# gongaa/video-layout-generation

Hardware: AMD Instinct MI355X
Metric: training clips/sec at (B,T,N)=(32,16,64) d=256; 1/2/4/8-GPU scaling (higher is better)
Workload: dtype f32

## Files before the change

include/vlg_hip.h:

```cpp
#ifndef VLG_HIP_H
#define VLG_HIP_H

#include <stdint.h>

typedef uint16_t vlg_bf16;

#ifdef __cplusplus
extern "C" {
#endif

#define VLG_ERR_SHAPE   1001
#define VLG_ERR_ALIGN   1002

int         vlg_abi_version(void);
const char* vlg_build_arch(void);

#ifdef VLG_DIAG
void vlg_debug_set_clock_probe(unsigned long long* buf);
void vlg_debug_set_conv_probe(unsigned long long* buf);
void vlg_debug_set_gemm_bk(int bk);
void vlg_debug_set_gemm_run(int run);
#endif

int vlg_embed_fwd(const int64_t* slot_class, const float* slot_box,
// ... 16 lines not shown
int vlg_layernorm_bwd(const float* dy, const float* x, const float* mean, const float* rstd,
                      const float* gamma, const float* dres, float* dx_out,
                      float* slabs, int64_t slab_stride, int64_t slab_capacity,
                      int64_t rows, int d, void* stream);
int vlg_layernorm_bwd_bf16(const vlg_bf16* dy, const float* x, const float* mean, const float* rstd,
                           const float* gamma, const float* dres, float* dx_out,
                           float* slabs, int64_t slab_stride, int64_t slab_capacity,
                           int64_t rows, int d, void* stream);

#define VLG_EPI_NONE   0
#define VLG_EPI_BIAS   1
#define VLG_EPI_GELU   2
#define VLG_EPI_RESID  4
#define VLG_EPI_DGELU  8
#define VLG_EPI_BF16   16
#define VLG_EPI_SPLIT3 256
#define VLG_EPI_ACT_GELU 512
#define VLG_EPI_GELU_GRAD 1024
#define VLG_EPI_MUL    2048
#define VLG_EPI_A_BF16   32
#define VLG_EPI_B_BF16   64
#define VLG_EPI_OUT_BF16 128
int vlg_linear_fwd(const void* A, int lda, const void* W, int ldw, const float* bias,
                   void* C, int ldc, const void* aux_in, void* aux_out,
                   int64_t M, int N, int K, int epilogue, void* stream);
int vlg_linear_dgrad(const void* dY, int ldy, const void* W, int ldw,
                     void* dX, int ldx, const void* aux_in,
                     int64_t M, int N, int K, int epilogue, void* stream);
int vlg_linear_wgrad_slabs(int64_t M, int N, int K);
int vlg_linear_wgrad_slabs_for(int64_t M, int N, int K, int flags);
int vlg_linear_wgrad(const void* dY, int ldy, const void* X, int ldx,
                     float* slabs, int64_t slab_stride, int64_t slab_capacity,
                     int64_t M, int N, int K, int flags , void* stream);
int vlg_linear_dgrad_wgrad(const void* dY, int ldy, const void* W, int ldw, void* dX, int ldx, const void* aux_in,
                           const void* X, int ldxx, float* slabs, int64_t slab_stride, int64_t slab_capacity,
                           int64_t M, int N, int K, int epilogue,
                           const int64_t* rider_table , int rider_rows, void* stream);


int vlg_attention_fwd(const float* qkv, float* o, int64_t n_seq, int T, int d, void* stream);
int vlg_attention_bwd(const float* qkv, const float* dout, float* dqkv,
                      int64_t n_seq, int T, int d, void* stream);
int vlg_attention_fwd_bf16(const vlg_bf16* qkv, vlg_bf16* o, int64_t n_seq, int T, int d, void* stream);
int vlg_attention_bwd_bf16(const vlg_bf16* qkv, const vlg_bf16* dout, vlg_bf16* dqkv,
                           int64_t n_seq, int T, int d, void* stream);

int vlg_layout_loss_scratch(void);
int vlg_layout_loss(const float* out, int ld, const int64_t* tgt_class, const float* tgt_box,
                    const float* valid, float* dout, float* loss_out, float* scratch,
                    int B, int T, int N, int n_classes, float beta, float iou_eps,
                    float w_reg, float w_iou, float w_ce, void* stream);

int vlg_attention_clip_fwd(const float* qkv, const float* valid, float* out, float* lse,
                           int64_t B, int T, int N, int d, void* stream);
int vlg_attention_clip_bwd(const float* qkv, const float* valid, const float* out, const float* dout, const float* lse,
                           float* delta, float* dqkv, int64_t B, int T, int N, int d, void* stream);
int vlg_attention_clip_fwd_bf16(const vlg_bf16* qkv, const float* valid, vlg_bf16* out, float* lse,
                                int64_t B, int T, int N, int d, void* stream);
int vlg_attention_clip_bwd_bf16(const vlg_bf16* qkv, const float* valid, const vlg_bf16* out, const vlg_bf16* dout,
                                const float* lse, float* delta, vlg_bf16* dqkv,
                                int64_t B, int T, int N, int d, void* stream);

int vlg_reduce_slabs(const float* slabs, int64_t slab_stride, int n_slabs,
                     float* dst, int64_t len, void* stream);

int vlg_adam_step_graph(float* param, const float* grad, float* exp_avg, float* exp_avg_sq, vlg_bf16* shadow,
// ... 101 lines not shown
```

video-layout-generation_amd/csrc/gemm.hip:

```cpp
#include "common.h"
#include <type_traits>

#include "gemm_tile.h"
#include "reduce_body.h"

#define GEMM_A_GELU (1 << 20)
#define GEMM_B_GELU (1 << 21)
__device__ __forceinline__ float4 gelu4(float4 v) { return make_float4(gelu_f(v.x), gelu_f(v.y), gelu_f(v.z), gelu_f(v.w)); }

__device__ __forceinline__ __amdgpu_buffer_rsrc_t vlg_rsrc(const void* p, int bytes = 0x7fffffff) {
    return __builtin_amdgcn_make_buffer_rsrc(const_cast<void*>(p), 0, bytes, 0x00020000);
}

#ifndef VLG_EPI_PACE
#define VLG_EPI_PACE 0
#endif
#ifndef VLG_EPI_PACE_EVERY
#define VLG_EPI_PACE_EVERY 2
#endif
__device__ __forceinline__ void vlg_epi_pace(int issued) {
#if VLG_EPI_PACE > 0
    if (issued % VLG_EPI_PACE_EVERY == 0) __builtin_amdgcn_s_sleep(VLG_EPI_PACE);
#endif
}

#ifdef VLG_NO_SCHED_FENCE
#define VLG_SCHED_FENCE()
#else
#define VLG_SCHED_FENCE() __builtin_amdgcn_sched_barrier(0)
#endif

template <int BM, int BN, int BK, bool A_KC, bool B_KC>
constexpr int gemm_smem_floats() { return 2 * (Tile<BM, A_KC, BK>::FLOATS + Tile<BN, B_KC, BK>::FLOATS); }

template <int BM, int BN, int BK, bool A_KC, bool B_KC, int EPI, bool COLSUM>
__device__ __forceinline__ void gemm_f32_body(const GemmArgs& g, float* const smem, const int bid, const int nwg) {
    __builtin_amdgcn_s_setprio(3);
    using EO = float;
    const float* const gA = static_cast<const float*>(g.A);
    const float* const gB = static_cast<const float*>(g.B);
    const float* const gAuxIn = static_cast<const float*>(g.aux_in);
    float* const gAuxOut = static_cast<float*>(g.aux_out);
    constexpr int WM = (BM == BN && (BM == 128 || BM == 64)) ? 2 : (BM == 128 ? 4 : 1);
    constexpr int WN = 4 / WM;
    constexpr int TM = BM / (32 * WM), TN = BN / (32 * WN);
    constexpr int NCH = BK / 8;
    using TA = Tile<BM, A_KC, BK>;
    using TB = Tile<BN, B_KC, BK>;
    float* const As0 = smem;
    float* const Bs0 = smem + 2 * TA::FLOATS;

    const int q = nwg >> 3, rr = nwg & 7, xcd = bid & 7;
    const int swz = (xcd < rr ? xcd * (q + 1) : rr * (q + 1) + (xcd - rr) * q) + (bid >> 3);
    constexpr bool CHAIN = BM == 128 && BN == 128 && BK == 32 && !COLSUM && (EPI & ((1 << 20) | (1 << 21))) == 0;
    const int run = (CHAIN && g.run > 1) ? g.run : 1;
    const int tng = g.tiles_n / run;
    const int ntile = g.tiles_m * tng;
    const int split = swz / ntile;
    const int tile = swz - split * ntile;
    const int tm = tile / tng, tn = (tile - tm * tng) * run;
    const int64_t m0 = (int64_t)tm * BM;
    const int n0 = tn * BN;
    const int64_t kbeg = (int64_t)split * g.kc_per_split;
    int64_t kend = kbeg + g.kc_per_split;
    if (kend > g.Kc) kend = g.Kc;

// ... 255 lines not shown
                if (GUARD && col0 + j * 32 >= g.N) continue;
                float aux[16];
                if constexpr ((EPI & (VLG_EPI_RESID | VLG_EPI_DGELU | VLG_EPI_MUL)) != 0) {
#pragma unroll
                    for (int r = 0; r < 16; ++r) {
                        const int ro = i * 32 + (r & 3) + 8 * (r >> 2);
                        aux[r] = (!GUARD || row0 + ro < g.M) ? ld1(gAuxIn + base + ro * g.ldc + j * 32) : 0.f;
                    }
                }
#pragma unroll
                for (int r = 0; r < 16; ++r) {
                    const int ro = i * 32 + (r & 3) + 8 * (r >> 2);
                    if (GUARD && row0 + ro >= g.M) continue;
                    const int64_t o = base + ro * g.ldc + j * 32;
                    float v = acc[i][j][r];
                    if constexpr ((EPI & VLG_EPI_GELU) != 0) {
                        if constexpr ((EPI & VLG_EPI_GELU_GRAD) != 0) {
                            float c, pd;
                            gelu_parts(v, c, pd);
                            st1(gAuxOut + o, c + v * pd);
                            v *= c;
                        } else {
                            st1(gAuxOut + o, v);
                            v = gelu_f(v);
                        }
                    }
                    if constexpr ((EPI & VLG_EPI_RESID) != 0) v += aux[r];
                    if constexpr ((EPI & VLG_EPI_DGELU) != 0) v *= dgelu_f(aux[r]);
                    if constexpr ((EPI & VLG_EPI_MUL) != 0) v *= aux[r];
                    st1(Cs + o, v);
                }
            }
    };
    auto emit_fast = [&](int n0v) __attribute__((always_inline)) {
        const int64_t corner = m0 * g.ldc + n0v;
        const __amdgpu_buffer_rsrc_t dc = vlg_rsrc(Cs + corner);
        const __amdgpu_buffer_rsrc_t dxin = vlg_rsrc(gAuxIn ? gAuxIn + corner : gA);
        const __amdgpu_buffer_rsrc_t dxout = vlg_rsrc(gAuxOut ? gAuxOut + corner : Cs + corner);
        const int vc = ((wm * TM * 32 + 4 * h) * g.ldc + wn * TN * 32 + l31) * 4;
        const int rowb = g.ldc * 4;
        constexpr bool AUX = (EPI & (VLG_EPI_RESID | VLG_EPI_DGELU | VLG_EPI_MUL)) != 0;
        constexpr bool AUX_ALL = BK == 32;
        constexpr int NAUX = AUX_ALL ? TM * TN : 2;
        float auxb[NAUX][16];
        auto fetch = [&](float (&a)[16], int i, int j) __attribute__((always_inline)) {
#pragma unroll
            for (int r = 0; r < 16; ++r) {
                a[r] = __uint_as_float(__builtin_amdgcn_raw_buffer_load_b32(dxin, vc + j * 128, (i * 32 + (r & 3) + 8 * (r >> 2)) * rowb, 0));
                vlg_epi_pace(r + 1);
            }
        };
        if constexpr (AUX) {
            if constexpr (AUX_ALL) {
#pragma unroll
                for (int t = 0; t < TM * TN; ++t) fetch(auxb[t], t / TN, t % TN);
            } else {
                fetch(auxb[0], 0, 0);
            }
        }
#pragma unroll
        for (int i = 0; i < TM; ++i)
#pragma unroll
            for (int j = 0; j < TN; ++j) {
                const int tix = i * TN + j;
                float (&aux)[16] = auxb[AUX_ALL ? tix : (tix & 1)];
                if constexpr (AUX && !AUX_ALL) {
                    if (tix + 1 < TM * TN) fetch(auxb[(tix + 1) & 1], (tix + 1) / TN, (tix + 1) % TN);
// ... 12 lines not shown
                        vlg_epi_pace(2 * q + 2);
                    }
                } else if constexpr ((EPI & VLG_EPI_GELU) != 0) {
#pragma unroll
                    for (int q = 0; q < 8; ++q) {
                        __builtin_amdgcn_raw_buffer_store_b32(__float_as_uint(v[q].x), dxout, vc + j * 128, soff(2 * q), 0);
                        __builtin_amdgcn_raw_buffer_store_b32(__float_as_uint(v[q].y), dxout, vc + j * 128, soff(2 * q + 1), 0);
                        vlg_epi_pace(2 * q + 2);
                    }
                    gelu2n<8>(v);
                }
                if constexpr ((EPI & VLG_EPI_RESID) != 0) {
#pragma unroll
                    for (int q = 0; q < 8; ++q) v[q] += v2f{aux[2 * q], aux[2 * q + 1]};
                }
                if constexpr ((EPI & VLG_EPI_MUL) != 0) {
#pragma unroll
                    for (int q = 0; q < 8; ++q) v[q] *= v2f{aux[2 * q], aux[2 * q + 1]};
                }
                if constexpr ((EPI & VLG_EPI_DGELU) != 0) {
                    v2f u[8], d[8];
#pragma unroll
                    for (int q = 0; q < 8; ++q) u[q] = v2f{aux[2 * q], aux[2 * q + 1]};
                    dgelu2n<8>(u, d);
#pragma unroll
                    for (int q = 0; q < 8; ++q) v[q] *= d[q];
                }
#pragma unroll
                for (int q = 0; q < 8; ++q) {
                    __builtin_amdgcn_raw_buffer_store_b32(__float_as_uint(v[q].x), dc, vc + j * 128, soff(2 * q), 0);
                    __builtin_amdgcn_raw_buffer_store_b32(__float_as_uint(v[q].y), dc, vc + j * 128, soff(2 * q + 1), 0);
                    vlg_epi_pace(2 * q + 2);
                }
            }
    };
    if (fast_tile) {
        for (int rt = 0; rt < run; ++rt) {
            const int n0v = n0 + rt * BN;
            const bool has_next = rt + 1 < run;
            mainloop_fast(n0v, rt == 0, has_next);
            if (has_next) load_bias(n0v + BN);
            emit_fast(n0v);
            if (has_next) init_acc();
        }
    } else if (full) emit(std::false_type{});
    else emit(std::true_type{});
#ifdef VLG_TIMELINE
    if (g.clock_probe) {
        asm volatile("s_waitcnt vmcnt(0)" ::: "memory");
        const unsigned long long tl_exit = __builtin_amdgcn_s_memrealtime();
        if (tid == 0) {
            unsigned long long* o = g.clock_probe + 8 * (size_t)bid;
            o[0] = tl_entry; o[1] = tl_loop0; o[2] = tl_loop1; o[3] = tl_exit;
            o[4] = __builtin_amdgcn_s_getreg(4 | (31 << 11));
            o[5] = __builtin_amdgcn_s_getreg(20 | (31 << 11));
            o[6] = (unsigned long long)tile; o[7] = (unsigned long long)split;
        }
    }
#endif
    if constexpr (COLSUM) {
        static_assert(!A_KC, "column sums are taken from a contraction-major A tile");
        if (tn == 0) {
            constexpr int PR = TA::PER_ROW, NG = GEMM_THREADS / PR;
            float* red = smem;
            st4(red + (tid / PR) * BM + 4 * (tid % PR), make_float4(col_lo.x, col_lo.y, col_hi.x, col_hi.y));
            __syncthreads();
            if (tid < BM && m0 + tid < g.M) {
                float s = 0.f;
#pragma unroll 8
                for (int t = 0; t < NG; ++t) s += red[t * BM + tid];
                st1(Cs + g.colsum_off + m0 + tid, s);
            }
        }
    }
}

template <int BM, int BN, int BK, bool A_KC, bool B_KC, int EPI, bool COLSUM>
__global__ __launch_bounds__(GEMM_THREADS, (BM == 64 && BN == 64) ? 4 : (BK == 16 ? 3 : 2)) void gemm_f32_kernel(const GemmArgs g) {
    __shared__ __attribute__((aligned(16))) float smem[gemm_smem_floats<BM, BN, BK, A_KC, B_KC>()];
    gemm_f32_body<BM, BN, BK, A_KC, B_KC, EPI, COLSUM>(g, smem, (int)blockIdx.x, (int)gridDim.x);
}

template <int BT, int EPI_D>
__global__ __launch_bounds__(GEMM_THREADS, BT == 64 ? 4 : 2) void gemm_pair_kernel(const GemmArgs gd, const GemmArgs gw, const int nd, const int nd_pad,
                                                                                   const int nw, const int64_t* __restrict__ rider, const int rider_bpr) {
    constexpr int FD = gemm_smem_floats<BT, BT, 32, true, false>(), FW = gemm_smem_floats<BT, BT, 32, false, false>();
    __shared__ __attribute__((aligned(16))) float smem_all[FD > FW ? FD : FW];
    const int b = (int)blockIdx.x;
    if (b < nd_pad) {
        if (b < nd) gemm_f32_body<BT, BT, 32, true, false, EPI_D, false>(gd, smem_all, b, nd);
    } else if (b < nd_pad + nw) {
        gemm_f32_body<BT, BT, 32, false, false, VLG_EPI_NONE, true>(gw, smem_all, b - nd_pad, nw);
    } else {
        const int rb = b - nd_pad - nw;
        reduce_table_row(rider, rb / rider_bpr, rb % rider_bpr, rider_bpr, reinterpret_cast<float4(*)[16]>(smem_all));
    }
}

#ifdef VLG_DIAG
static unsigned long long* vlg_gemm_clock_probe = nullptr;
extern "C" void vlg_debug_set_clock_probe(unsigned long long* p) { vlg_gemm_clock_probe = p; }
#else
static constexpr unsigned long long* vlg_gemm_clock_probe = nullptr;
#endif

#ifdef VLG_DIAG
static int vlg_gemm_bk_forced = -1;
extern "C" void vlg_debug_set_gemm_bk(int bk) { vlg_gemm_bk_forced = (bk == 16 || bk == 32) ? bk : 0; }
#endif
static int gemm_bk_override() {
#ifdef VLG_DIAG
    if (vlg_gemm_bk_forced >= 0) return vlg_gemm_bk_forced;
#endif
    return VLG_TUNE("VLG_GEMM_BK", 0);
}

#ifdef VLG_DIAG
static int vlg_gemm_run_forced = -1;
extern "C" void vlg_debug_set_gemm_run(int run) { vlg_gemm_run_forced = run < 0 ? -1 : run; }
#else
static constexpr int vlg_gemm_run_forced = -1;
#endif
template <int BM, int BN, int BK, bool A_KC, bool B_KC>
static int gemm_run(const GemmArgs& g, int slots) {
    if (BM != 128 || BN != 128 || g.splits != 1) return 1;
    if (g.M % BM != 0 || g.N % BN != 0 || g.Kc % (2 * BK) != 0) return 1;
    const int64_t span_a = A_KC ? (int64_t)(BM - 1) * g.lda + g.Kc : g.Kc * g.lda + BM;
    const int64_t span_b = B_KC ? (int64_t)(2 * BN - 1) * g.ldb + g.Kc : g.Kc * g.ldb + 2 * BN;
    if (span_a >= (1ll << 28) || span_b >= (1ll << 28) || (int64_t)(BM - 1) * g.ldc + BN >= (1ll << 28)) return 1;
    if (vlg_gemm_run_forced == 0) return 1;
    int best = 1;
    for (int r = 2; r <= g.tiles_n; ++r)
        if (g.tiles_n % r == 0 && (int64_t)g.tiles_m * (g.tiles_n / r) >= slots) best = r;
    if (vlg_gemm_run_forced > 0 && g.tiles_n % vlg_gemm_run_forced == 0) best = vlg_gemm_run_forced;
    return best;
}

static bool gemm_small_tiles() { return VLG_TUNE("VLG_GEMM_SMALL", 1) != 0; }
static int gemm_small_below() { return VLG_TUNE("VLG_GEMM_SMALL_BELOW", 512); }
static int gemm_small_below_wgrad() { return VLG_TUNE("VLG_GEMM_SMALL_BELOW_WGRAD", 385); }
static bool gemm_wants_small(int64_t M, int N, int splits) {
    return gemm_small_tiles() && ((M + 127) / 128) * (int64_t)((N + 127) / 128) * splits < gemm_small_below();
}

template <int BM, int BN, bool A_KC, bool B_KC, int EPI, bool COLSUM>
static int launch_gemm(GemmArgs g, hipStream_t s) {
    if constexpr (BM == 128 && BN == 128 && !COLSUM && (EPI & (GEMM_A_GELU | GEMM_B_GELU)) == 0) {
        if (gemm_wants_small(g.M, g.N, g.splits)) return launch_gemm<64, 64, A_KC, B_KC, EPI, COLSUM>(g, s);
    }
    g.tiles_m = (int)((g.M + BM - 1) / BM);
    g.tiles_n = (g.N + BN - 1) / BN;
    g.run = 1;
    g.clock_probe = vlg_gemm_clock_probe;
    const dim3 block(GEMM_THREADS);
    constexpr bool CAN_RUN = BM == 128 && BN == 128 && !COLSUM && (EPI & (GEMM_A_GELU | GEMM_B_GELU)) == 0;
    if constexpr (BM == 128 && BN == 128) {
        const int forced = gemm_bk_override();
        const bool heavy_epilogue = (EPI & (VLG_EPI_GELU | VLG_EPI_DGELU)) != 0;
        int run32 = 1;
        if constexpr (CAN_RUN) run32 = gemm_run<BM, BN, 32, A_KC, B_KC>(g, 512);
        if (forced == 16 || (forced != 32 && heavy_epilogue && run32 == 1)) {
            const int64_t blocks = (int64_t)g.tiles_m * (g.tiles_n / g.run) * g.splits;
// ... 40 lines not shown
    if ((epilogue & VLG_EPI_BIAS) && !bias) return VLG_ERR_SHAPE;
    if ((epilogue & (VLG_EPI_RESID | VLG_EPI_DGELU)) && !aux_in) return VLG_ERR_SHAPE;
    if ((epilogue & VLG_EPI_GELU) && !aux_out) return VLG_ERR_SHAPE;
    if ((epilogue & VLG_EPI_MUL) != 0) return VLG_ERR_SHAPE;
    if ((epilogue & VLG_EPI_GELU_GRAD) && (split3 || epilogue != (VLG_EPI_BIAS | VLG_EPI_GELU | VLG_EPI_GELU_GRAD)))
        return VLG_ERR_SHAPE;
    const bool narrow = N <= 32;
    const bool act_gelu = (epilogue & VLG_EPI_ACT_GELU) != 0;
    epilogue &= ~VLG_EPI_ACT_GELU;
    if (act_gelu && (bf16 || split3)) return VLG_ERR_SHAPE;
    if (io != 0 && !bf16) return VLG_ERR_SHAPE;
    if (((io & 1) && (lda & 7)) || ((io & 2) && (ldw & 7))) return VLG_ERR_ALIGN;
    if (bf16) return vlg_gemm16_fwd(g, epilogue, io, s);
    if (split3) return vlg_gemm_split_fwd(g, epilogue, s);
    if (act_gelu) {
        if (epilogue != (VLG_EPI_BIAS | VLG_EPI_RESID) || narrow) return VLG_ERR_SHAPE;
        return launch_gemm<128, 128, true, true, VLG_EPI_BIAS | VLG_EPI_RESID | GEMM_A_GELU, false>(g, s);
    }
    switch (epilogue) {
        case VLG_EPI_BIAS:
            return narrow ? launch_gemm<128, 32, true, true, VLG_EPI_BIAS, false>(g, s)
                          : launch_gemm<128, 128, true, true, VLG_EPI_BIAS, false>(g, s);
        case VLG_EPI_BIAS | VLG_EPI_GELU:
            return launch_gemm<128, 128, true, true, VLG_EPI_BIAS | VLG_EPI_GELU, false>(g, s);
        case VLG_EPI_BIAS | VLG_EPI_GELU | VLG_EPI_GELU_GRAD:
            return launch_gemm<128, 128, true, true, VLG_EPI_BIAS | VLG_EPI_GELU | VLG_EPI_GELU_GRAD, false>(g, s);
        case VLG_EPI_BIAS | VLG_EPI_RESID:
            return launch_gemm<128, 128, true, true, VLG_EPI_BIAS | VLG_EPI_RESID, false>(g, s);
        default:
            return VLG_ERR_SHAPE;
    }
}

static int check_dgrad(const void* dY, int ldy, const void* W, int ldw, const void* dX, int ldx, const void* aux_in,
                       int64_t M, int N, int K, int flags) {
    if (M < 1 || N < 4 || (N & 3) || K < 4 || (K & 3) || ldy < N || ldw < K || ldx < K) return VLG_ERR_SHAPE;
    if (!gemm_ptr_ok(dY, ldy) || !gemm_ptr_ok(W, ldw) || !dX) return VLG_ERR_ALIGN;
    const bool bf16 = (flags & VLG_EPI_BF16) != 0, split3 = (flags & VLG_EPI_SPLIT3) != 0;
    const int io = gemm_io_bits(flags);
    const int epi = flags & ~(VLG_EPI_BF16 | VLG_EPI_STORAGE | VLG_EPI_SPLIT3);
    if (split3 && (bf16 || io != 0)) return VLG_ERR_SHAPE;
    if (io != 0 && !bf16) return VLG_ERR_SHAPE;
    if (((io & 1) && (ldy & 7)) || ((io & 2) && (ldw & 7))) return VLG_ERR_ALIGN;
    if ((epi == VLG_EPI_DGELU || epi == VLG_EPI_MUL) && !aux_in) return VLG_ERR_SHAPE;
    if (epi == VLG_EPI_MUL && split3) return VLG_ERR_SHAPE;
    return 0;
}
static int check_wgrad(const void* dY, int ldy, const void* X, int ldx, const float* slabs, int64_t slab_stride,
                       int64_t M, int N, int K, int flags) {
    if (M < 1 || N < 4 || (N & 3) || K < 4 || (K & 3) || ldy < N || ldx < K) return VLG_ERR_SHAPE;
    if (slab_stride < (int64_t)N * K + N) return VLG_ERR_SHAPE;
    if (!gemm_ptr_ok(dY, ldy) || !gemm_ptr_ok(X, ldx) || !slabs) return VLG_ERR_ALIGN;
    const int io = gemm_io_bits(flags);
    if (io != 0 && !(flags & VLG_EPI_BF16)) return VLG_ERR_SHAPE;
    if (((io & 1) && (ldy & 7)) || ((io & 2) && (ldx & 7))) return VLG_ERR_ALIGN;
    return 0;
}

static GemmArgs dgrad_args(const void* dY, int ldy, const void* W, int ldw, void* dX, int ldx, const void* aux_in, int64_t M, int N, int K) {
    GemmArgs g{};
    g.A = dY; g.B = W; g.C = dX; g.aux_in = aux_in;
    g.M = M; g.N = K; g.Kc = N; g.lda = ldy; g.ldb = ldw; g.ldc = ldx;
    g.splits = 1; g.kc_per_split = N;
    return g;
}

// ... 134 lines not shown
```

video-layout-generation_amd/csrc/gemm_tile.h:

```cpp
#pragma once
#include "common.h"

typedef float f32x16 __attribute__((ext_vector_type(16)));
typedef __bf16 bf16x8 __attribute__((ext_vector_type(8)));

#define GEMM_THREADS 256

struct GemmArgs {
    const void* A; const void* B; void* C;
    const float* bias; const void* aux_in; void* aux_out;
    int64_t M;
    int N;
    int64_t Kc;
    int lda, ldb, ldc;
    int tiles_m, tiles_n, splits;
    int run;
    int64_t kc_per_split, slab_stride, colsum_off;
    unsigned long long* clock_probe;
};

template <int N_MFMA, int N_ST, int N_LD>
__device__ __forceinline__ void pin_staging() {
    constexpr int PER = (N_ST + N_LD + N_MFMA - 1) / N_MFMA;
#pragma unroll
    for (int i = 0; i < N_MFMA; ++i) {
        __builtin_amdgcn_sched_group_barrier(0x008, 1, 0);
#pragma unroll
        for (int q = 0; q < PER; ++q) {
            const int slot = i * PER + q;
            if (slot < N_ST) __builtin_amdgcn_sched_group_barrier(0x200, 1, 0);
            else if (slot < N_ST + N_LD) __builtin_amdgcn_sched_group_barrier(0x020, 1, 0);
        }
    }
}


template <int BR, bool KC, int BK, int NT = GEMM_THREADS>
struct Tile {
    static constexpr int LDK = BK + 4;
    static constexpr int F4 = BR * BK / 4;
    static constexpr int NV = (F4 + NT - 1) / NT;
    static constexpr int FLOATS = KC ? BR * LDK : BK * BR;
    static constexpr int PER_ROW = KC ? BK / 4 : BR / 4;

    template <bool GUARD, typename E>
    __device__ static __forceinline__ void gload(float4 (&r)[NV], const E* __restrict__ P, int ld,
                                                 int64_t r0, int64_t R, int64_t k0, int64_t kend, int tid) {
#pragma unroll
        for (int i = 0; i < NV; ++i) {
            const int idx = tid + NT * i;
            if (F4 % NT != 0 && idx >= F4) { r[i] = f4_zero(); continue; }
// ... 48 lines not shown
```

video-layout-generation_amd/csrc/layernorm.hip:

```cpp
#include "common.h"

#define LN_BLOCK 256
#define LN_WAVES (LN_BLOCK / 64)
#define LN_BWD_MAX_BLOCKS 512

template <int E, bool V4>
struct RowIO {
    template <typename EL>
    __device__ static __forceinline__ void load(const EL* __restrict__ row, int lane, float (&v)[E]) {
        if constexpr (V4) {
#pragma unroll
            for (int i = 0; i < E / 4; ++i) {
                const float4 t = ld4(row + 4 * lane + 256 * i);
                v[4 * i] = t.x; v[4 * i + 1] = t.y; v[4 * i + 2] = t.z; v[4 * i + 3] = t.w;
            }
        } else {
#pragma unroll
            for (int i = 0; i < E; ++i) v[i] = ld1(row + lane + 64 * i);
        }
    }
    template <typename EL>
    __device__ static __forceinline__ void store(EL* __restrict__ row, int lane, const float (&v)[E]) {
        if constexpr (V4) {
#pragma unroll
            for (int i = 0; i < E / 4; ++i)
                st4(row + 4 * lane + 256 * i, make_float4(v[4 * i], v[4 * i + 1], v[4 * i + 2], v[4 * i + 3]));
        } else {
#pragma unroll
            for (int i = 0; i < E; ++i) st1(row + lane + 64 * i, v[i]);
        }
    }
    __device__ static __forceinline__ int col(int lane, int j) {
        if constexpr (V4) return 4 * lane + 256 * (j >> 2) + (j & 3);
        else return lane + 64 * j;
    }
};

#define LN_ROWS(E) ((E) <= 4 ? 4 : (E) <= 8 ? 2 : 1)

template <int E, bool V4, typename EY = float>
__global__ __launch_bounds__(LN_BLOCK) void ln_fwd_kernel(
    const float* __restrict__ x, const float* __restrict__ gamma, const float* __restrict__ beta,
    EY* __restrict__ y, float* __restrict__ mean, float* __restrict__ rstd, int64_t rows, float eps) {
    constexpr int d = E * 64, R = LN_ROWS(E);
    const int lane = threadIdx.x & 63;
    const int64_t wave = (int64_t)blockIdx.x * LN_WAVES + (threadIdx.x >> 6);
    const int64_t nwaves = (int64_t)gridDim.x * LN_WAVES;
    float g[E], b[E];
    RowIO<E, V4>::load(gamma, lane, g);
    RowIO<E, V4>::load(beta, lane, b);
    for (int64_t r0 = wave * R; r0 < rows; r0 += nwaves * R) {
        float v[R][E];
#pragma unroll
        for (int i = 0; i < R; ++i) {
            const int64_t r = r0 + i < rows ? r0 + i : rows - 1;
            RowIO<E, V4>::load(x + r * d, lane, v[i]);
        }
#pragma unroll
        for (int i = 0; i < R; ++i) {
            float s = 0.f;
#pragma unroll
            for (int j = 0; j < E; ++j) s += v[i][j];
            const float mu = wave_sum(s) * (1.0f / d);
            float q = 0.f;
#pragma unroll
            for (int j = 0; j < E; ++j) { const float t = v[i][j] - mu; q += t * t; }
            const float rs = 1.0f / sqrtf(wave_sum(q) * (1.0f / d) + eps);
#pragma unroll
            for (int j = 0; j < E; ++j) v[i][j] = (v[i][j] - mu) * rs * g[j] + b[j];
            if (r0 + i < rows) {
                RowIO<E, V4>::store(y + (r0 + i) * d, lane, v[i]);
                if (lane == 0) { mean[r0 + i] = mu; rstd[r0 + i] = rs; }
            }
        }
    }
}

template <int E, bool V4, typename EY = float>
__global__ __launch_bounds__(LN_BLOCK) void ln_bwd_kernel(
    const EY* __restrict__ dy, const float* __restrict__ x, const float* __restrict__ mean,
    const float* __restrict__ rstd, const float* __restrict__ gamma, const float* __restrict__ dres,
    float* __restrict__ dx_out, float* __restrict__ slabs, int64_t slab_stride, int64_t rows) {
    constexpr int d = E * 64, R = LN_ROWS(E);
    __shared__ float red[LN_WAVES][2 * d];
    const int lane = threadIdx.x & 63, w = threadIdx.x >> 6;
    const int64_t wave = (int64_t)blockIdx.x * LN_WAVES + w;
    const int64_t nwaves = (int64_t)gridDim.x * LN_WAVES;
    float g[E], dg[E], db[E];
    RowIO<E, V4>::load(gamma, lane, g);
#pragma unroll
    for (int j = 0; j < E; ++j) { dg[j] = 0.f; db[j] = 0.f; }
    for (int64_t r0 = wave * R; r0 < rows; r0 += nwaves * R) {
        float gy[R][E], xv[R][E], o[R][E], mu[R], rs[R];
#pragma unroll
        for (int i = 0; i < R; ++i) {
            const int64_t r = r0 + i < rows ? r0 + i : rows - 1;
            RowIO<E, V4>::load(dy + r * d, lane, gy[i]);
            RowIO<E, V4>::load(x + r * d, lane, xv[i]);
            if (dres != nullptr) RowIO<E, V4>::load(dres + r * d, lane, o[i]);
            else {
#pragma unroll
                for (int j = 0; j < E; ++j) o[i][j] = 0.f;
            }
            mu[i] = mean[r];
            rs[i] = rstd[r];
// ... 119 lines not shown
```

video-layout-generation_amd/vlg/engine.py:

```python
from __future__ import annotations

import math
import os
from typing import Dict, Optional

import torch

from . import hip
from .hip import (EPI_A_BF16, EPI_B_BF16, EPI_BIAS, EPI_DGELU, EPI_GELU, EPI_NONE, EPI_OUT_BF16, EPI_RESID,
                  call, ptr)
from .spec import (ADAM_BETA1, ADAM_BETA2, ADAM_EPS, ADAM_LR, BOX_DIM, IOU_EPS, LN_EPS, LOSS_W_CE,
                   LOSS_W_REG, LOSS_W_STRUCT, SMOOTH_L1_BETA, LayoutConfig, param_layout)


def init_params(cfg: LayoutConfig, seed: int) -> Dict[str, torch.Tensor]:
    layout, _ = param_layout(cfg)
    g = torch.Generator().manual_seed(seed)
    fan_in = {name[:-2] + "_b": shape[1] for name, (_, shape) in layout.items() if name.endswith("_w")}
    out: Dict[str, torch.Tensor] = {}
    for name, (_, shape) in layout.items():
        base = name.split(".")[-1]
        if base in ("cls_emb", "time_emb"):
            t = torch.randn(shape, generator=g, dtype=torch.float32)
        elif base.endswith("_g"):
# ... 280 lines not shown
            return
        self._timed("attn_fwd", 0.0, "vlg_attention_fwd" + self._sfx, ptr(self.qkv[l]), ptr(self.att[l]), B * N, T, d, s,
                    nbytes=4.0 * self.qkv.element_size() * M * d)

    def _attn_bwd(self, l: int, batch, B, T, N, M) -> None:
        d, s = self.cfg.d, self._stream()
        if self.cfg.attention == "clip":
            fl = 2.5 * 4.0 * B * d * N * N * T * (T + 1) / 2.0
            e = self.qkv.element_size()
            self._timed("attn_clip_bwd", fl, "vlg_attention_clip_bwd" + self._sfx, ptr(self.qkv[l]),
                        ptr(batch["valid"]) if self.padded_slots else 0, ptr(self.att[l]), ptr(self.dh), ptr(self.lse[l]),
                        ptr(self.delta), ptr(self.dqkv), B, T, N, d, s, nbytes=7.0 * e * M * d)
            return
        self._timed("attn_bwd", 0.0, "vlg_attention_bwd" + self._sfx, ptr(self.qkv[l]), ptr(self.dh), ptr(self.dqkv), B * N, T, d, s,
                    nbytes=7.0 * self.qkv.element_size() * M * d)

    def _ln_fwd(self, x, gname, y, stat, M):
        d = self.cfg.d
        self._timed("ln_fwd", 0.0, "vlg_layernorm_fwd_bf16" if y.dtype == torch.bfloat16 else "vlg_layernorm_fwd", ptr(x), ptr(self.p(gname)),
                    ptr(self.p(gname[:-1] + "b")), ptr(y), ptr(stat[0]), ptr(stat[1]), M, d, LN_EPS, self._stream(),
                    nbytes=(4.0 + y.element_size()) * M * d)

    def _ln_bwd(self, dy, x, stat, gname, dres, dx_out, M):
        d = self.cfg.d
        lib = hip.load()
        n_slabs = lib.vlg_layernorm_bwd_slabs(M)
        arena = self._arena("s", n_slabs * 2 * d)
        s = self._stream()
        self._timed("ln_bwd", 0.0, "vlg_layernorm_bwd_bf16" if dy.dtype == torch.bfloat16 else "vlg_layernorm_bwd", ptr(dy), ptr(x), ptr(stat[0]),
                    ptr(stat[1]), ptr(self.p(gname)), ptr(dres), ptr(dx_out), ptr(arena), 2 * d, arena.numel(), M, d, s,
                    nbytes=(dy.element_size() + 4.0 + 4.0 + (4.0 if dres is not None else 0.0)) * M * d)
        self._reduce("s", 2 * d, n_slabs, self.layout[gname][0], 2 * d)

    def _check_batch(self, batch) -> tuple:
        sc = batch["slot_class"]
        B, T, N = sc.shape
        if T != self.cfg.T:
            raise ValueError("batch has T=%d, engine was built for T=%d" % (T, self.cfg.T))
        M = B * T * N
        if M > self.capacity:
            raise ValueError("batch of %d tokens exceeds workspace capacity %d" % (M, self.capacity))
        for k, dt in (("slot_class", torch.int64), ("slot_box", torch.float32), ("tgt_class", torch.int64),
                      ("tgt_box", torch.float32), ("valid", torch.float32)):
            t = batch[k]
            if t.dtype != dt or not t.is_cuda or not t.is_contiguous():
                raise ValueError("batch[%r] must be a contiguous %s HIP tensor" % (k, dt))
        return B, T, N, M

    def forward(self, batch: Dict[str, torch.Tensor]) -> torch.Tensor:
        cfg, d, ff = self.cfg, self.cfg.d, self.cfg.d_ff
        B, T, N, M = self._check_batch(batch)
        self._shape = (B, T, N, M)
        s = self._stream()
        self._timed("embed_fwd", 0.0, "vlg_embed_fwd", ptr(batch["slot_class"]), ptr(batch["slot_box"]), ptr(self.p("cls_emb")),
                    ptr(self.p("box_w")), ptr(self.p("box_b")), ptr(self.p("time_emb")), ptr(self.x[0]),
                    B, T, N, d, cfg.vocab, s, nbytes=4.0 * M * d + 24.0 * M)
        for l in range(cfg.n_layers):
            pre = "l%d." % l
            x = self.x[l]
            self._ln_fwd(x, pre + "ln1_g", self.h1[l], self.stats[2 * l], M)
            self._linear(self.h1[l], self.pw(pre + "qkv_w"), self.p(pre + "qkv_b"), self.qkv[l], M, 3 * d, d, EPI_BIAS)
            self._attn_fwd(l, batch, B, T, N, M)
            self._linear(self.att[l], self.pw(pre + "proj_w"), self.p(pre + "proj_b"), self.xmid[l], M, d, d,
                         EPI_BIAS | EPI_RESID, aux_in=x)
            self._ln_fwd(self.xmid[l], pre + "ln2_g", self.h2[l], self.stats[2 * l + 1], M)
            self._linear(self.h2[l], self.pw(pre + "ff1_w"), self.p(pre + "ff1_b"), self.gl[l], M, ff, d,
                         self._epi_ff1, aux_out=self.u[l])
            self._linear(self.gl[l], self.pw(pre + "ff2_w"), self.p(pre + "ff2_b"), self.x[l + 1], M, d, ff,
                         EPI_BIAS | EPI_RESID, aux_in=self.xmid[l])
        L = cfg.n_layers
        self._ln_fwd(self.x[L], "lnf_g", self.xf, self.stats[2 * L], M)
        self._linear(self.xf, self.pw("head_w"), self.p("head_b"), self.out, M, cfg.n_out, d, EPI_BIAS)
        self._timed("loss", 0.0, "vlg_layout_loss", ptr(self.out), cfg.n_out, ptr(batch["tgt_class"]), ptr(batch["tgt_box"]),
                    ptr(batch["valid"]), ptr(self.dout), ptr(self.loss_out), ptr(self.loss_scratch), B, T, N,
                    cfg.n_classes, SMOOTH_L1_BETA, IOU_EPS, LOSS_W_REG, LOSS_W_STRUCT, LOSS_W_CE, s,
                    nbytes=(2.0 * 4 * cfg.n_out + 8 + 16 + 4) * M)
        return self.loss_out

    def backward(self, batch: Dict[str, torch.Tensor], reducer=None) -> None:
        cfg, d, ff = self.cfg, self.cfg.d, self.cfg.d_ff
        B, T, N, M = self._shape
        main = torch.cuda.current_stream(self.device)
        side = self.side if self.overlap_wgrad else main
        s = main.cuda_stream
        L = cfg.n_layers
        last_read: Dict[str, torch.cuda.Event] = {}

        def on_side(reads, fn):
            if side is main:
                fn()
                return
            e = torch.cuda.Event()
            e.record(main)
            side.wait_event(e)
            with torch.cuda.stream(side):
                fn()
                done = torch.cuda.Event()
                done.record(side)
            for name in reads:
                last_read[name] = done

        def before_write(*names):
            for name in names:
                e = last_read.pop(name, None)
# ... 180 lines not shown
```

video-layout-generation_amd/vlg/hip.py:

```python
from __future__ import annotations

import ctypes
import os
from ctypes import c_char_p, c_float, c_int, c_int64, c_void_p

_HERE = os.path.dirname(os.path.abspath(__file__))
LIB_PATH = os.environ.get("VLG_HIP_LIB") or os.path.join(os.path.dirname(_HERE), "libvlg_hip.so")

EPI_NONE, EPI_BIAS, EPI_GELU, EPI_RESID, EPI_DGELU, EPI_BF16 = 0, 1, 2, 4, 8, 16
EPI_A_BF16, EPI_B_BF16, EPI_OUT_BF16, EPI_SPLIT3 = 32, 64, 128, 256
EPI_ACT_GELU = 512
EPI_GELU_GRAD, EPI_MUL = 1024, 2048

P, I, L, F = c_void_p, c_int, c_int64, c_float

SIGNATURES = {
    "vlg_abi_version": (I, []),
    "vlg_build_arch": (c_char_p, []),
    "vlg_embed_fwd": (I, [P, P, P, P, P, P, P, I, I, I, I, I, P]),
    "vlg_embed_bwd_slabs": (I, []),
    "vlg_embed_bwd_slabs_for": (I, [I, I, I, I, I]),
    "vlg_embed_bwd": (I, [P, P, P, P, L, L, I, I, I, I, I, P]),
    "vlg_layernorm_fwd": (I, [P, P, P, P, P, P, L, I, F, P]),
    "vlg_layernorm_fwd_bf16": (I, [P, P, P, P, P, P, L, I, F, P]),
    "vlg_layernorm_bwd_slabs": (I, [L]),
    "vlg_layernorm_bwd": (I, [P, P, P, P, P, P, P, P, L, L, L, I, P]),
    "vlg_layernorm_bwd_bf16": (I, [P, P, P, P, P, P, P, P, L, L, L, I, P]),
    "vlg_linear_fwd": (I, [P, I, P, I, P, P, I, P, P, L, I, I, I, P]),
    "vlg_linear_dgrad": (I, [P, I, P, I, P, I, P, L, I, I, I, P]),
    "vlg_linear_wgrad_slabs": (I, [L, I, I]),
    "vlg_linear_dgrad_wgrad": (I, [P, I, P, I, P, I, P, P, I, P, L, L, L, I, I, I, P, I, P]),
    "vlg_linear_wgrad_slabs_for": (I, [L, I, I, I]),
    "vlg_linear_wgrad": (I, [P, I, P, I, P, L, L, L, I, I, I, P]),
    "vlg_attention_fwd": (I, [P, P, L, I, I, P]),
    "vlg_attention_bwd": (I, [P, P, P, L, I, I, P]),
    "vlg_attention_fwd_bf16": (I, [P, P, L, I, I, P]),
    "vlg_attention_bwd_bf16": (I, [P, P, P, L, I, I, P]),
    "vlg_attention_clip_fwd": (I, [P, P, P, P, L, I, I, I, P]),
    "vlg_attention_clip_bwd": (I, [P, P, P, P, P, P, P, L, I, I, I, P]),
    "vlg_attention_clip_fwd_bf16": (I, [P, P, P, P, L, I, I, I, P]),
    "vlg_attention_clip_bwd_bf16": (I, [P, P, P, P, P, P, P, L, I, I, I, P]),
    "vlg_layout_loss_scratch": (I, []),
    "vlg_layout_loss": (I, [P, I, P, P, P, P, P, P, I, I, I, I, F, F, F, F, F, P]),
    "vlg_reduce_slabs": (I, [P, L, I, P, L, P]),
    "vlg_reduce_slabs_table": (I, [P, I, I, P]),
    "vlg_sum_partials_table": (I, [P, I, P]),
    "vlg_adam_step": (I, [P, P, P, P, L, I, F, F, F, F, F, P]),
    "vlg_adam_step_graph": (I, [P, P, P, P, P, L, P, I, F, F, F, F, F, P]),
    "vlg_adam_step_bf16": (I, [P, P, P, P, P, L, I, F, F, F, F, F, P]),
    "vlg_image_loss_scratch": (I, []),
    "vlg_ce_nchw": (I, [P, P, P, P, P, I, I, L, F, P]),
    "vlg_l1_mean": (I, [P, P, P, P, P, L, F, P]),
    "vlg_gradient_loss": (I, [P, P, P, P, P, I, I, I, F, P]),
    "vlg_ssim_loss": (I, [P, P, P, P, P, I, I, I, I, F, P]),
    "vlg_affine_nchw": (I, [P, P, I, I, L, P, P, P]),
    "vlg_prep_input": (I, [P, P, P, P, P, P, P, P, P, P, P, I, I, I, I, P]),
    "vlg_argmax_nchw": (I, [P, P, I, I, L, P]),
    "vlg_rollout_input": (I, [P, P, P, P, P, P, P, I, L, P]),
    "vlg_conv3x3_fwd": (I, [P, P, P, P, P, P, P, P, L, I, I, I, I, I, I, P, L, P]),
    "vlg_conv3x3_fwd_splits": (I, [L, I, I, I]),
    "vlg_conv3x3_fwd_workspace": (L, [L, I, I, I]),
# ... 108 lines not shown
```

Before: 5871.

## Fuse LayerNorm into residual GEMM epilogue for proj and ff2 linears

Adds a GEMM variant whose epilogue, after writing bias+residual output, parks each 128x256 row block in LDS and runs LayerNorm over it, writing normalized output plus mean/rstd. The forward pass now uses it after the attention projection and after ff2, which removes separate LayerNorm launches and their re-read of the activations. A shared row-LN helper with a permlane/DPP wave reduction also replaces the inline code in the standalone LN kernel. The cost is a larger LDS footprint for the fused kernel, which can lower occupancy, and an extra barrier before the LN pass.

```diff
diff --git a/include/vlg_hip.h b/include/vlg_hip.h
--- a/include/vlg_hip.h
+++ b/include/vlg_hip.h
@@ -72,6 +72,10 @@
 int vlg_linear_wgrad(const void* dY, int ldy, const void* X, int ldx,
                      float* slabs, int64_t slab_stride, int64_t slab_capacity,
                      int64_t M, int N, int K, int flags , void* stream);
+int vlg_linear_fwd_ln_ok(int64_t M, int N, int K);
+int vlg_linear_fwd_ln(const float* A, int lda, const float* W, int ldw, const float* bias, float* C, const float* resid,
+                      const float* gamma, const float* beta, float* y, float* mean, float* rstd,
+                      int64_t M, int N, int K, float eps, void* stream);
 int vlg_linear_dgrad_wgrad(const void* dY, int ldy, const void* W, int ldw, void* dX, int ldx, const void* aux_in,
                            const void* X, int ldxx, float* slabs, int64_t slab_stride, int64_t slab_capacity,
                            int64_t M, int N, int K, int epilogue,
diff --git a/video-layout-generation_amd/csrc/gemm.hip b/video-layout-generation_amd/csrc/gemm.hip
--- a/video-layout-generation_amd/csrc/gemm.hip
+++ b/video-layout-generation_amd/csrc/gemm.hip
@@ -2,10 +2,14 @@
 #include <type_traits>
 
 #include "gemm_tile.h"
+#include "ln_row.h"
 #include "reduce_body.h"
 
 #define GEMM_A_GELU (1 << 20)
 #define GEMM_B_GELU (1 << 21)
+#define GEMM_LN (1 << 22)
+#define GEMM_LN_LD 132
+#define GEMM_LN_PARK (128 * GEMM_LN_LD)
 __device__ __forceinline__ float4 gelu4(float4 v) { return make_float4(gelu_f(v.x), gelu_f(v.y), gelu_f(v.z), gelu_f(v.w)); }
 
 __device__ __forceinline__ __amdgpu_buffer_rsrc_t vlg_rsrc(const void* p, int bytes = 0x7fffffff) {
@@ -32,6 +36,11 @@
 
 template <int BM, int BN, int BK, bool A_KC, bool B_KC>
 constexpr int gemm_smem_floats() { return 2 * (Tile<BM, A_KC, BK>::FLOATS + Tile<BN, B_KC, BK>::FLOATS); }
+template <int BM, int BN, int BK, bool A_KC, bool B_KC, int EPI>
+constexpr int gemm_kernel_smem_floats() {
+    constexpr int F = gemm_smem_floats<BM, BN, BK, A_KC, B_KC>();
+    return (EPI & GEMM_LN) == 0 ? F : (F > GEMM_LN_PARK ? F : GEMM_LN_PARK) + GEMM_LN_PARK;
+}
 
 template <int BM, int BN, int BK, bool A_KC, bool B_KC, int EPI, bool COLSUM>
 __device__ __forceinline__ void gemm_f32_body(const GemmArgs& g, float* const smem, const int bid, const int nwg) {
@@ -353,7 +362,11 @@
                 }
             }
     };
-    auto emit_fast = [&](int n0v) __attribute__((always_inline)) {
+    constexpr bool LN = (EPI & GEMM_LN) != 0;
+    static_assert(!LN || (CHAIN && FAST && BM == 128 && (EPI & VLG_EPI_RESID) != 0), "the layer-norm epilogue runs on the chained fast path");
+    float* const park_first = smem + (gemm_smem_floats<BM, BN, BK, A_KC, B_KC>() > GEMM_LN_PARK ? gemm_smem_floats<BM, BN, BK, A_KC, B_KC>() : GEMM_LN_PARK);
+    float* const park_last = smem;
+    auto emit_fast = [&](int n0v, float* park) __attribute__((always_inline)) {
         const int64_t corner = m0 * g.ldc + n0v;
         const __amdgpu_buffer_rsrc_t dc = vlg_rsrc(Cs + corner);
         const __amdgpu_buffer_rsrc_t dxin = vlg_rsrc(gAuxIn ? gAuxIn + corner : gA);
@@ -432,7 +445,40 @@
                     __builtin_amdgcn_raw_buffer_store_b32(__float_as_uint(v[q].y), dc, vc + j * 128, soff(2 * q + 1), 0);
                     vlg_epi_pace(2 * q + 2);
                 }
-            }
+                if constexpr (LN) {
+                    float* const pw = park + (wm * TM * 32 + i * 32 + 4 * h) * GEMM_LN_LD + wn * TN * 32 + j * 32 + l31;
+                    const auto prow = [](int r) { return ((r & 3) + 8 * (r >> 2)) * GEMM_LN_LD; };
+#pragma unroll
+                    for (int q = 0; q < 8; ++q) {
+                        pw[prow(2 * q)] = v[q].x;
+                        pw[prow(2 * q + 1)] = v[q].y;
+                    }
+                }
+            }
+    };
+    auto ln_pass = [&]() __attribute__((always_inline)) {
+        constexpr int LR = 16;
+        const float* const src = (lane < 32 ? park_first : park_last) + 4 * (lane & 31);
+        float gm[4], bt[4];
+        const float4 tg = ld4(g.ln_gamma + 4 * lane), tb = ld4(g.ln_beta + 4 * lane);
+        gm[0] = tg.x; gm[1] = tg.y; gm[2] = tg.z; gm[3] = tg.w;
+        bt[0] = tb.x; bt[1] = tb.y; bt[2] = tb.z; bt[3] = tb.w;
+#pragma unroll
+        for (int r0 = wave * 32; r0 < wave * 32 + 32; r0 += LR) {
+            float v[LR][4], mu[LR], rs[LR];
+#pragma unroll
+            for (int i = 0; i < LR; ++i) {
+                const float4 t = ld4(src + (r0 + i) * GEMM_LN_LD);
+                v[i][0] = t.x; v[i][1] = t.y; v[i][2] = t.z; v[i][3] = t.w;
+            }
+            ln_rows_fwd<4, LR>(v, gm, bt, g.ln_eps, mu, rs);
+#pragma unroll
+            for (int i = 0; i < LR; ++i) {
+                const int64_t row = m0 + r0 + i;
+                st4(g.ln_y + row * 256 + 4 * lane, make_float4(v[i][0], v[i][1], v[i][2], v[i][3]));
+                if (lane == 0) { g.ln_mean[row] = mu[i]; g.ln_rstd[row] = rs[i]; }
+            }
+        }
     };
     if (fast_tile) {
         for (int rt = 0; rt < run; ++rt) {
@@ -440,8 +486,13 @@
             const bool has_next = rt + 1 < run;
             mainloop_fast(n0v, rt == 0, has_next);
             if (has_next) load_bias(n0v + BN);
-            emit_fast(n0v);
+            if (LN && !has_next) __syncthreads();
+            emit_fast(n0v, has_next ? park_first : park_last);
             if (has_next) init_acc();
+        }
+        if constexpr (LN) {
+            __syncthreads();
+            ln_pass();
         }
     } else if (full) emit(std::false_type{});
     else emit(std::true_type{});
@@ -477,7 +528,7 @@
 
 template <int BM, int BN, int BK, bool A_KC, bool B_KC, int EPI, bool COLSUM>
 __global__ __launch_bounds__(GEMM_THREADS, (BM == 64 && BN == 64) ? 4 : (BK == 16 ? 3 : 2)) void gemm_f32_kernel(const GemmArgs g) {
-    __shared__ __attribute__((aligned(16))) float smem[gemm_smem_floats<BM, BN, BK, A_KC, B_KC>()];
+    __shared__ __attribute__((aligned(16))) float smem[gemm_kernel_smem_floats<BM, BN, BK, A_KC, B_KC, EPI>()];
     gemm_f32_body<BM, BN, BK, A_KC, B_KC, EPI, COLSUM>(g, smem, (int)blockIdx.x, (int)gridDim.x);
 }
 
@@ -522,12 +573,16 @@
 static constexpr int vlg_gemm_run_forced = -1;
 #endif
 template <int BM, int BN, int BK, bool A_KC, bool B_KC>
-static int gemm_run(const GemmArgs& g, int slots) {
-    if (BM != 128 || BN != 128 || g.splits != 1) return 1;
-    if (g.M % BM != 0 || g.N % BN != 0 || g.Kc % (2 * BK) != 0) return 1;
+static bool gemm_can_chain(const GemmArgs& g) {
+    if (BM != 128 || BN != 128 || g.splits != 1) return false;
+    if (g.M % BM != 0 || g.N % BN != 0 || g.Kc % (2 * BK) != 0) return false;
     const int64_t span_a = A_KC ? (int64_t)(BM - 1) * g.lda + g.Kc : g.Kc * g.lda + BM;
     const int64_t span_b = B_KC ? (int64_t)(2 * BN - 1) * g.ldb + g.Kc : g.Kc * g.ldb + 2 * BN;
-    if (span_a >= (1ll << 28) || span_b >= (1ll << 28) || (int64_t)(BM - 1) * g.ldc + BN >= (1ll << 28)) return 1;
+    return span_a < (1ll << 28) && span_b < (1ll << 28) && (int64_t)(BM - 1) * g.ldc + BN < (1ll << 28);
+}
+template <int BM, int BN, int BK, bool A_KC, bool B_KC>
+static int gemm_run(const GemmArgs& g, int slots) {
+    if (!gemm_can_chain<BM, BN, BK, A_KC, B_KC>(g)) return 1;
     if (vlg_gemm_run_forced == 0) return 1;
     int best = 1;
     for (int r = 2; r <= g.tiles_n; ++r)
@@ -634,6 +689,39 @@
     }
 }
 
+static GemmArgs fwd_ln_args(const float* A, int lda, const float* W, int ldw, const float* bias, float* C, const float* resid,
+                            int64_t M, int N, int K) {
+    GemmArgs g{};
+    g.A = A; g.B = W; g.C = C; g.bias = bias; g.aux_in = resid;
+    g.M = M; g.N = N; g.Kc = K; g.lda = lda; g.ldb = ldw; g.ldc = N;
+    g.splits = 1; g.kc_per_split = K;
+    g.tiles_m = (int)((M + 127) / 128); g.tiles_n = (N + 127) / 128; g.run = g.tiles_n;
+    return g;
+}
+static bool fwd_ln_plan_ok(const GemmArgs& g) {
+    return g.N == 256 && g.M >= 128 && g.M % 128 == 0 && g.M / 128 <= 0x7fffffff && !gemm_wants_small(g.M, g.N, 1) &&
+           gemm_can_chain<128, 128, 32, true, true>(g);
+}
+extern "C" int vlg_linear_fwd_ln_ok(int64_t M, int N, int K) {
+    if (M < 1 || N < 1 || K < 4 || (K & 3)) return 0;
+    return fwd_ln_plan_ok(fwd_ln_args(nullptr, K, nullptr, K, nullptr, nullptr, nullptr, M, N, K)) ? 1 : 0;
+}
+extern "C" int vlg_linear_fwd_ln(const float* A, int lda, const float* W, int ldw, const float* bias, float* C, const float* resid,
+                                 const float* gamma, const float* beta, float* y, float* mean, float* rstd,
+                                 int64_t M, int N, int K, float eps, void* stream) {
+    if (M < 1 || N < 1 || K < 4 || (K & 3) || lda < K || ldw < K) return VLG_ERR_SHAPE;
+    if (!bias || !C || !resid || !gamma || !beta || !y || !mean || !rstd) return VLG_ERR_SHAPE;
+    if (!gemm_ptr_ok(A, lda) || !gemm_ptr_ok(W, ldw) || !vlg_aligned16(C) || !vlg_aligned16(resid) || !vlg_aligned16(gamma) ||
+        !vlg_aligned16(beta) || !vlg_aligned16(y)) return VLG_ERR_ALIGN;
+    GemmArgs g = fwd_ln_args(A, lda, W, ldw, bias, C, resid, M, N, K);
+    if (!fwd_ln_plan_ok(g)) return VLG_ERR_SHAPE;
+    g.ln_gamma = gamma; g.ln_beta = beta; g.ln_y = y; g.ln_mean = mean; g.ln_rstd = rstd; g.ln_eps = eps;
+    g.clock_probe = vlg_gemm_clock_probe;
+    hipLaunchKernelGGL((gemm_f32_kernel<128, 128, 32, true, true, VLG_EPI_BIAS | VLG_EPI_RESID | GEMM_LN, false>), dim3((unsigned)g.tiles_m),
+                       dim3(GEMM_THREADS), 0, (hipStream_t)stream, g);
+    return vlg_last_error();
+}
+
 static int check_dgrad(const void* dY, int ldy, const void* W, int ldw, const void* dX, int ldx, const void* aux_in,
                        int64_t M, int N, int K, int flags) {
     if (M < 1 || N < 4 || (N & 3) || K < 4 || (K & 3) || ldy < N || ldw < K || ldx < K) return VLG_ERR_SHAPE;
diff --git a/video-layout-generation_amd/csrc/gemm_tile.h b/video-layout-generation_amd/csrc/gemm_tile.h
--- a/video-layout-generation_amd/csrc/gemm_tile.h
+++ b/video-layout-generation_amd/csrc/gemm_tile.h
@@ -17,6 +17,7 @@
     int run;
     int64_t kc_per_split, slab_stride, colsum_off;
     unsigned long long* clock_probe;
+    const float* ln_gamma; const float* ln_beta; float* ln_y; float* ln_mean; float* ln_rstd; float ln_eps;
 };
 
 template <int N_MFMA, int N_ST, int N_LD>
diff --git a/video-layout-generation_amd/csrc/layernorm.hip b/video-layout-generation_amd/csrc/layernorm.hip
--- a/video-layout-generation_amd/csrc/layernorm.hip
+++ b/video-layout-generation_amd/csrc/layernorm.hip
@@ -1,4 +1,5 @@
 #include "common.h"
+#include "ln_row.h"
 
 #define LN_BLOCK 256
 #define LN_WAVES (LN_BLOCK / 64)
@@ -56,21 +57,13 @@
             const int64_t r = r0 + i < rows ? r0 + i : rows - 1;
             RowIO<E, V4>::load(x + r * d, lane, v[i]);
         }
-#pragma unroll
-        for (int i = 0; i < R; ++i) {
-            float s = 0.f;
-#pragma unroll
-            for (int j = 0; j < E; ++j) s += v[i][j];
-            const float mu = wave_sum(s) * (1.0f / d);
-            float q = 0.f;
-#pragma unroll
-            for (int j = 0; j < E; ++j) { const float t = v[i][j] - mu; q += t * t; }
-            const float rs = 1.0f / sqrtf(wave_sum(q) * (1.0f / d) + eps);
-#pragma unroll
-            for (int j = 0; j < E; ++j) v[i][j] = (v[i][j] - mu) * rs * g[j] + b[j];
+        float mu[R], rs[R];
+        ln_rows_fwd<E, R>(v, g, b, eps, mu, rs);
+#pragma unroll
+        for (int i = 0; i < R; ++i) {
             if (r0 + i < rows) {
                 RowIO<E, V4>::store(y + (r0 + i) * d, lane, v[i]);
-                if (lane == 0) { mean[r0 + i] = mu; rstd[r0 + i] = rs; }
+                if (lane == 0) { mean[r0 + i] = mu[i]; rstd[r0 + i] = rs[i]; }
             }
         }
     }
diff --git a/video-layout-generation_amd/csrc/ln_row.h b/video-layout-generation_amd/csrc/ln_row.h
--- /dev/null
+++ b/video-layout-generation_amd/csrc/ln_row.h
@@ -0,0 +1,54 @@
+#pragma once
+#include "common.h"
+
+template <int CTRL>
+__device__ __forceinline__ float ln_dpp_step(float v) {
+    return v + __int_as_float(__builtin_amdgcn_update_dpp(0, __float_as_int(v), CTRL, 0xf, 0xf, false));
+}
+__device__ __forceinline__ float ln_wave_sum(float v) {
+    const unsigned u32 = __float_as_uint(v);
+    const auto s32 = __builtin_amdgcn_permlane32_swap(u32, u32, false, false);
+    v = __uint_as_float(s32[0]) + __uint_as_float(s32[1]);
+    const unsigned u16 = __float_as_uint(v);
+    const auto s16 = __builtin_amdgcn_permlane16_swap(u16, u16, false, false);
+    v = __uint_as_float(s16[0]) + __uint_as_float(s16[1]);
+    v = ln_dpp_step<0x128>(v);
+    v = ln_dpp_step<0x124>(v);
+    v = ln_dpp_step<0x4e>(v);
+    v = ln_dpp_step<0xb1>(v);
+    return v;
+}
+
+template <int E, int R>
+__device__ __forceinline__ void ln_rows_fwd(float (&v)[R][E], const float (&g)[E], const float (&b)[E], float eps,
+                                            float (&mu)[R], float (&rs)[R]) {
+    static_assert(R <= 64, "one lane per row");
+    constexpr int d = E * 64;
+#pragma unroll
+    for (int i = 0; i < R; ++i) {
+        float s = 0.f;
+#pragma unroll
+        for (int j = 0; j < E; ++j) s += v[i][j];
+        mu[i] = ln_wave_sum(s) * (1.0f / d);
+    }
+    const int lane = threadIdx.x & 63;
+    float qs = 0.f;
+#pragma unroll
+    for (int i = 0; i < R; ++i) {
+        float q = 0.f;
+        {
+#pragma clang fp contract(off)
+#pragma unroll
+            for (int j = 0; j < E; ++j) { const float t = v[i][j] - mu[i]; q += t * t; }
+        }
+        q = ln_wave_sum(q);
+        qs = lane == i ? q : qs;
+    }
+    const int r = __float_as_int(1.0f / sqrtf(qs * (1.0f / d) + eps));
+#pragma unroll
+    for (int i = 0; i < R; ++i) {
+        rs[i] = __int_as_float(__builtin_amdgcn_readlane(r, i));
+#pragma unroll
+        for (int j = 0; j < E; ++j) v[i][j] = (v[i][j] - mu[i]) * rs[i] * g[j] + b[j];
+    }
+}
diff --git a/video-layout-generation_amd/vlg/engine.py b/video-layout-generation_amd/vlg/engine.py
--- a/video-layout-generation_amd/vlg/engine.py
+++ b/video-layout-generation_amd/vlg/engine.py
@@ -336,6 +336,16 @@
                     nbytes=(dy.element_size() + 4.0 + 4.0 + (4.0 if dres is not None else 0.0)) * M * d)
         self._reduce("s", 2 * d, n_slabs, self.layout[gname][0], 2 * d)
 
+    def _linear_ln(self, a, w, b, c, M, K, resid, gname, y, stat):
+        d = self.cfg.d
+        if self.precision != "fp32" or not hip.load().vlg_linear_fwd_ln_ok(M, d, K):
+            self._linear(a, w, b, c, M, d, K, EPI_BIAS | EPI_RESID, aux_in=resid)
+            self._ln_fwd(c, gname, y, stat, M)
+            return
+        self._timed("gemm_fwd", 2.0 * M * d * K, "vlg_linear_fwd_ln", ptr(a), K, ptr(w), K, ptr(b), ptr(c), ptr(resid),
+                    ptr(self.p(gname)), ptr(self.p(gname[:-1] + "b")), ptr(y), ptr(stat[0]), ptr(stat[1]), M, d, K, LN_EPS,
+                    self._stream(), nbytes=4.0 * (M * K + d * K + 4 * M * d))
+
     def _check_batch(self, batch) -> tuple:
         sc = batch["slot_class"]
         B, T, N = sc.shape
@@ -359,21 +369,19 @@
         self._timed("embed_fwd", 0.0, "vlg_embed_fwd", ptr(batch["slot_class"]), ptr(batch["slot_box"]), ptr(self.p("cls_emb")),
                     ptr(self.p("box_w")), ptr(self.p("box_b")), ptr(self.p("time_emb")), ptr(self.x[0]),
                     B, T, N, d, cfg.vocab, s, nbytes=4.0 * M * d + 24.0 * M)
-        for l in range(cfg.n_layers):
+        L = cfg.n_layers
+        self._ln_fwd(self.x[0], "l0.ln1_g", self.h1[0], self.stats[0], M)
+        for l in range(L):
             pre = "l%d." % l
             x = self.x[l]
-            self._ln_fwd(x, pre + "ln1_g", self.h1[l], self.stats[2 * l], M)
             self._linear(self.h1[l], self.pw(pre + "qkv_w"), self.p(pre + "qkv_b"), self.qkv[l], M, 3 * d, d, EPI_BIAS)
             self._attn_fwd(l, batch, B, T, N, M)
-            self._linear(self.att[l], self.pw(pre + "proj_w"), self.p(pre + "proj_b"), self.xmid[l], M, d, d,
-                         EPI_BIAS | EPI_RESID, aux_in=x)
-            self._ln_fwd(self.xmid[l], pre + "ln2_g", self.h2[l], self.stats[2 * l + 1], M)
+            self._linear_ln(self.att[l], self.pw(pre + "proj_w"), self.p(pre + "proj_b"), self.xmid[l], M, d, x,
+                            pre + "ln2_g", self.h2[l], self.stats[2 * l + 1])
             self._linear(self.h2[l], self.pw(pre + "ff1_w"), self.p(pre + "ff1_b"), self.gl[l], M, ff, d,
                          self._epi_ff1, aux_out=self.u[l])
-            self._linear(self.gl[l], self.pw(pre + "ff2_w"), self.p(pre + "ff2_b"), self.x[l + 1], M, d, ff,
-                         EPI_BIAS | EPI_RESID, aux_in=self.xmid[l])
-        L = cfg.n_layers
-        self._ln_fwd(self.x[L], "lnf_g", self.xf, self.stats[2 * L], M)
+            nxt = ("l%d.ln1_g" % (l + 1), self.h1[l + 1], self.stats[2 * l + 2]) if l + 1 < L else ("lnf_g", self.xf, self.stats[2 * L])
+            self._linear_ln(self.gl[l], self.pw(pre + "ff2_w"), self.p(pre + "ff2_b"), self.x[l + 1], M, ff, self.xmid[l], *nxt)
         self._linear(self.xf, self.pw("head_w"), self.p("head_b"), self.out, M, cfg.n_out, d, EPI_BIAS)
         self._timed("loss", 0.0, "vlg_layout_loss", ptr(self.out), cfg.n_out, ptr(batch["tgt_class"]), ptr(batch["tgt_box"]),
                     ptr(batch["valid"]), ptr(self.dout), ptr(self.loss_out), ptr(self.loss_scratch), B, T, N,
diff --git a/video-layout-generation_amd/vlg/hip.py b/video-layout-generation_amd/vlg/hip.py
--- a/video-layout-generation_amd/vlg/hip.py
+++ b/video-layout-generation_amd/vlg/hip.py
@@ -27,6 +27,8 @@
     "vlg_layernorm_bwd": (I, [P, P, P, P, P, P, P, P, L, L, L, I, P]),
     "vlg_layernorm_bwd_bf16": (I, [P, P, P, P, P, P, P, P, L, L, L, I, P]),
     "vlg_linear_fwd": (I, [P, I, P, I, P, P, I, P, P, L, I, I, I, P]),
+    "vlg_linear_fwd_ln_ok": (I, [L, I, I]),
+    "vlg_linear_fwd_ln": (I, [P, I, P, I, P, P, P, P, P, P, P, P, L, I, I, F, P]),
     "vlg_linear_dgrad": (I, [P, I, P, I, P, I, P, L, I, I, I, P]),
     "vlg_linear_wgrad_slabs": (I, [L, I, I]),
     "vlg_linear_dgrad_wgrad": (I, [P, I, P, I, P, I, P, P, I, P, L, L, L, I, I, I, P, I, P]),
```

Result: no change. 5899 (median of 6 runs) (+0.5%).
